# nwihardjo/SpaghettiSearch

Hardware: AMD Instinct MI355X
Metric: pagerank_iters_per_sec (higher is better)
Workload: dtype f64

## Files before the change

### include/spaghetti_rank.h

```cpp
#ifndef SPAGHETTI_RANK_H
#define SPAGHETTI_RANK_H

#include <stdint.h>

#ifdef __cplusplus
extern "C" {
#endif

#define SS_ABI_VERSION 4

enum {
    SS_OK = 0,
    SS_ERR_INVALID = 1,
    SS_ERR_NO_DEVICE = 2,
    SS_ERR_HIP = 3,
    SS_ERR_OOM = 4,
    SS_ERR_UNSORTED = 5,
    SS_ERR_STATE = 6,
    SS_ERR_UNSUPPORTED = 7,
    SS_ERR_COMM = 8
};

#define SS_MAX_TOPK 1024
#define SS_MAX_TOPICS 64
// ... 96 lines not shown
                       float* w_out, double* mag_out, float* idf_out);
int32_t ss_index_set_doc_freq(ss_index* idx, const uint64_t* df );
int32_t ss_index_set_weighted(ss_index* idx, const double* mag );
int32_t ss_index_set_positions(ss_index* idx, const uint64_t* pos_ptr, const float* pos);

int32_t ss_index_apply_delta(ss_index* idx, uint64_t n_del_docs, const uint32_t* del_docs,
                             uint64_t n_del, const uint32_t* del_term, const uint32_t* del_doc,
                             uint64_t n_add, const uint32_t* add_term, const uint32_t* add_doc, const float* add_w);
int32_t ss_index_apply_delta_pos(ss_index* idx, uint64_t n_del_docs, const uint32_t* del_docs,
                                 uint64_t n_del, const uint32_t* del_term, const uint32_t* del_doc,
                                 uint64_t n_add, const uint32_t* add_term, const uint32_t* add_doc, const float* add_w,
                                 const uint64_t* add_pos_ptr , const float* add_pos);
int32_t ss_index_resize(ss_index* idx, uint64_t n_docs_new, uint64_t n_terms_new);
int32_t ss_index_read_magnitudes(ss_index* idx, uint64_t n, const uint32_t* docs, double* mag_out);
int32_t ss_index_refresh_magnitudes(ss_index* idx, double* mag_out);
int32_t ss_index_get_info(const ss_index* idx, uint64_t* n_docs, uint64_t* n_terms, uint64_t* n_post);
int32_t ss_index_read(ss_index* idx, uint64_t* term_ptr_out , uint32_t* post_doc_out, float* post_w_out);
int32_t ss_index_read_positions(ss_index* idx, uint64_t* pos_ptr_out, float* pos_out);

int32_t ss_index_build_doc_view(ss_index* idx);
int32_t ss_index_drop_doc_view(ss_index* idx);
int32_t ss_index_read_doc_view(ss_index* idx, uint64_t* doc_ptr_out, uint32_t* doc_term_out, float* doc_w_out);
int32_t ss_index_doc_top_terms(ss_index* idx, uint64_t n, const uint32_t* docs , int32_t m,
                               uint32_t* terms_out , float* w_out , int32_t* n_out );

int32_t ss_scorer_create(ss_ctx* ctx, ss_index* title, ss_index* body, ss_scorer** out);
int32_t ss_scorer_destroy(ss_scorer* s);
int32_t ss_scorer_set_prior(ss_scorer* s, int32_t k_topics, const double* rank);
int32_t ss_score_topk(ss_scorer* s, int32_t n_q, const uint32_t* q_ptr, const uint32_t* q_terms,
                      const int32_t* query_len, const double* topic_probs, int32_t k,
// ... 196 lines not shown
```

### spaghettisearch_amd/_lib.py

```python
from __future__ import annotations

import ctypes as C
import os

_HERE = os.path.dirname(os.path.abspath(__file__))
LIB_PATH = os.environ.get("SS_LIB_PATH") or os.path.join(_HERE, "libspaghetti_rank.so")

SS_OK = 0
SS_MAX_TOPK = 1024
SS_MAX_TOPICS = 64
SS_MAX_QUERY_TERMS = 64
SS_MAX_FEEDBACK_DOCS = 64
SS_UNKNOWN_TERM = 0xFFFFFFFF
SS_NO_GROUP = 0xFFFFFFFF
SS_MAX_WORD_BYTES = 64
SS_MAX_EDIT_DIST = 3
SS_MAX_SUGGEST = 64
SS_MAX_SIG_SLOTS = 32
SS_SIG_EMPTY = 0xFFFFFFFF
SS_MAX_LINKS = 64
SS_LINKS_PARENTS = 0
SS_LINKS_CHILDREN = 1
SS_MAX_DOC_FIELDS = 4
SS_MAX_RANGE_CLAUSES = 4
# ... 95 lines not shown
    "ss_pr_exchange": (_i32, [_vp, _i32]),
    "ss_pagerank_run_sharded": (_i32, [_vp, _f64, _f64, _i32, _i32, _vp, _i32, _vp, _vp, _vp]),
    "ss_pagerank_run_group": (_i32, [_vp, _i32, _f64, _f64, _i32, _i32, _vp, _vp, _vp]),
    "ss_pr_status": (_i32, [_vp, _vp, C.POINTER(_i32), C.POINTER(_i32), _vp, _vp]),
    "ss_pr_read_local": (_i32, [_vp, _vp, _vp]),
    "ss_pr_read": (_i32, [_vp, _vp]),
    "ss_pr_probe": (_i32, [_vp, _i32, _i32, C.POINTER(C.c_float)]),
    "ss_index_create": (_i32, [_vp, _u64, _u64, _vp, _vp, _vp, C.POINTER(_vp)]),
    "ss_index_destroy": (_i32, [_vp]),
    "ss_tfidf_build": (_i32, [_vp, _u64, _vp, _vp, _vp]),
    "ss_index_apply_delta": (_i32, [_vp, _u64, _vp, _u64, _vp, _vp, _u64, _vp, _vp, _vp]),
    "ss_index_apply_delta_pos": (_i32, [_vp, _u64, _vp, _u64, _vp, _vp, _u64, _vp, _vp, _vp, _vp, _vp]),
    "ss_index_resize": (_i32, [_vp, _u64, _u64]),
    "ss_index_read_magnitudes": (_i32, [_vp, _u64, _vp, _vp]),
    "ss_index_refresh_magnitudes": (_i32, [_vp, _vp]),
    "ss_index_get_info": (_i32, [_vp, C.POINTER(_u64), C.POINTER(_u64), C.POINTER(_u64)]),
    "ss_index_read": (_i32, [_vp, _vp, _vp, _vp]),
    "ss_index_read_positions": (_i32, [_vp, _vp, _vp]),
    "ss_index_set_doc_freq": (_i32, [_vp, _vp]),
    "ss_index_set_weighted": (_i32, [_vp, _vp]),
    "ss_index_set_positions": (_i32, [_vp, _vp, _vp]),
    "ss_index_build_doc_view": (_i32, [_vp]),
    "ss_index_drop_doc_view": (_i32, [_vp]),
    "ss_index_read_doc_view": (_i32, [_vp, _vp, _vp, _vp]),
    "ss_index_doc_top_terms": (_i32, [_vp, _u64, _vp, _i32, _vp, _vp, _vp]),
    "ss_scorer_create": (_i32, [_vp, _vp, _vp, C.POINTER(_vp)]),
    "ss_scorer_destroy": (_i32, [_vp]),
    "ss_scorer_set_prior": (_i32, [_vp, _i32, _vp]),
    "ss_score_topk": (_i32, [_vp, _i32, _vp, _vp, _vp, _vp, _i32, _vp, _vp]),
    "ss_score_topk_phrase": (_i32, [_vp, _i32, _vp, _vp, _vp, _vp, _vp, _vp, _i32, _vp, _vp]),
# ... 76 lines not shown
```

### spaghettisearch_amd/csrc/ctx.hip

```cpp
#include "common.hpp"
#include <chrono>

#include <unordered_map>

namespace ss {

namespace {
struct Pool {
    std::mutex mu;
    std::multimap<std::pair<int, size_t>, void*> free_blocks;
    std::unordered_map<void*, std::pair<int, size_t>> live;
    size_t held = 0, limit = (size_t)64 << 30;
    double miss_ms = 0.0;
    uint64_t misses = 0;
    int contexts = 0;
};
Pool& pool() { static Pool* p = new Pool(); return *p; }
size_t size_class(size_t b) {
    if (b <= 4096) return 4096;
    size_t p2 = 4096;
    while (p2 < b) p2 <<= 1;
    if (p2 <= ((size_t)1 << 20)) return p2;
    const size_t step = p2 >> 4;
    return (b + step - 1) / step * step;
// ... 257 lines not shown
    "pr.lean_sweeps",
    "pr.item_turns",
    "graph.late_free",
    "graph.readback_runs",
    "pr.trace",
    "score.collect_pinned",
    "score.pipeline_slices",
    "score.timing",
    "score.trace",
    "pr.probe_hot",
    "pr.topic_blocks",
    "tfidf.blocks",
    "tfidf.bucket_shift",
    "tfidf.head_min_run",
    "tfidf.bucket_min",
    "score.wave",
    "score.wave_max_terms",
    "score.wave_min_list",
    "score.wave_share_pct",
    "score.wave_slice_target",
    "score.wave_big_pct",
    "score.wave_big_x100",
    "score.small",
    "score.small_max_batch",
    "score.small_batch",
    "score.small_cap",
    "score.pipeline",
    "score.grade_slices",
    "score.wave_small_x100",
    "score.exact_all",
// ... 55 lines not shown
```

### spaghettisearch_amd/csrc/index.hip

```cpp
#include "index.hpp"
#include <algorithm>
#include <memory>
#include <new>

namespace {

constexpr int TPB = 256;

__global__ void k_check_ptr(const uint64_t* __restrict__ term_ptr, uint64_t n_terms, const uint32_t* __restrict__ post_doc,
                            unsigned long long* __restrict__ n_boundary_desc, uint32_t* __restrict__ err) {
    const uint64_t t = (uint64_t)blockIdx.x * blockDim.x + threadIdx.x;
    if (t >= n_terms) return;
    const uint64_t a = term_ptr[t], b = term_ptr[t + 1];
    if (b < a) { atomicOr(err, 1u); return; }
    if (b > a && a > 0 && post_doc[a] <= post_doc[a - 1]) atomicAdd(n_boundary_desc, 1ull);
}
__global__ void k_check_df(const uint64_t* __restrict__ term_ptr, const uint64_t* __restrict__ df, uint64_t n_terms,
                           uint32_t* __restrict__ err) {
    const uint64_t t = (uint64_t)blockIdx.x * blockDim.x + threadIdx.x;
    if (t >= n_terms) return;
    if (df[t] < term_ptr[t + 1] - term_ptr[t]) atomicOr(err, 1u);
}
__global__ void k_check_pos(const uint64_t* __restrict__ pos_ptr, uint64_t n_post, uint32_t* __restrict__ err) {
    uint64_t i = (uint64_t)blockIdx.x * blockDim.x + threadIdx.x;
// ... 54 lines not shown
    SS_HIP(ctx, idx->mag2.alloc(n_docs));
    if (P) {
        SS_HIP(ctx, hipMemcpyAsync(idx->post_doc.p, post_doc, P * sizeof(uint32_t), hipMemcpyDefault, st));
        SS_HIP(ctx, hipMemcpyAsync(idx->post_w.p, post_tf, P * sizeof(float), hipMemcpyDefault, st));
    }
    SS_HIP(ctx, hipMemsetAsync(idx->mag.p, 0, n_docs * sizeof(double), st));

    ss::DevBuf<unsigned long long> d_cnt;
    ss::DevBuf<uint32_t> d_err;
    SS_HIP(ctx, d_cnt.alloc(2));
    SS_HIP(ctx, d_err.alloc(1));
    SS_HIP(ctx, hipMemsetAsync(d_cnt.p, 0, 2 * sizeof(unsigned long long), st));
    SS_HIP(ctx, hipMemsetAsync(d_err.p, 0, sizeof(uint32_t), st));
    if (n_terms) hipLaunchKernelGGL(k_check_ptr, dim3(ss::div_up(n_terms, TPB)), dim3(TPB), 0, st, idx->term_ptr.p, n_terms,
                                    idx->post_doc.p, d_cnt.p, d_err.p);
    if (P) hipLaunchKernelGGL(k_check_docs, dim3(std::min<unsigned>(ss::div_up(P, TPB), 16384u)), dim3(TPB), 0, st,
                              idx->post_doc.p, P, n_docs, d_cnt.p + 1, d_err.p);
    unsigned long long h_cnt[2] = {0, 0};
    uint32_t h_err = 0;
    SS_HIP(ctx, ss::fetch(ctx, st, h_cnt, d_cnt.p, sizeof(h_cnt), &h_err, d_err.p, sizeof(h_err)));
    SS_HIP(ctx, hipGetLastError());
    if (h_err & 1) return ctx->fail(SS_ERR_INVALID, "ss_index_create: term_ptr is not non-decreasing");
    if (h_err & 2) return ctx->fail(SS_ERR_INVALID, "ss_index_create: posting holds a doc id >= n_docs");
    if (h_cnt[1] != h_cnt[0])
        return ctx->fail(SS_ERR_UNSORTED, "ss_index_create: %llu posting(s) not strictly ascending by doc id inside a term",
                         h_cnt[1] - h_cnt[0]);
    *out = idx.release();
    return SS_OK;
}

int32_t ss_index_destroy(ss_index* idx) {
    if (!idx) return SS_ERR_INVALID;
// ... 2 lines not shown
    if (idx->users > 0) return ctx->fail(SS_ERR_STATE, "ss_index_destroy: index still used by %d scorer(s)", idx->users);
    (void)hipSetDevice(ctx->device);
    (void)hipStreamSynchronize(ctx->stream);
    delete idx;
    return SS_OK;
}

int32_t ss_index_get_info(const ss_index* idx, uint64_t* n_docs, uint64_t* n_terms, uint64_t* n_post) {
    if (!idx) return SS_ERR_INVALID;
    if (n_docs) *n_docs = idx->n_docs;
    if (n_terms) *n_terms = idx->n_terms;
    if (n_post) *n_post = idx->n_post;
    return SS_OK;
}

int32_t ss_index_read(ss_index* idx, uint64_t* term_ptr_out, uint32_t* post_doc_out, float* post_w_out) {
    if (!idx) return SS_ERR_INVALID;
    ss_ctx* ctx = idx->ctx;
    std::lock_guard<std::recursive_mutex> lk(ctx->mu);
    SS_HIP(ctx, hipSetDevice(ctx->device));
    hipStream_t st = ctx->stream;
    if (term_ptr_out) SS_HIP(ctx, hipMemcpyAsync(term_ptr_out, idx->term_ptr.p, (idx->n_terms + 1) * sizeof(uint64_t), hipMemcpyDefault, st));
    if (post_doc_out && idx->n_post) SS_HIP(ctx, hipMemcpyAsync(post_doc_out, idx->post_doc.p, idx->n_post * sizeof(uint32_t), hipMemcpyDefault, st));
    if (post_w_out && idx->n_post) SS_HIP(ctx, hipMemcpyAsync(post_w_out, idx->post_w.p, idx->n_post * sizeof(float), hipMemcpyDefault, st));
    SS_HIP(ctx, hipStreamSynchronize(st));
    return SS_OK;
}

int32_t ss_index_read_positions(ss_index* idx, uint64_t* pos_ptr_out, float* pos_out) {
    if (!idx) return SS_ERR_INVALID;
// ... 1 lines not shown
    std::lock_guard<std::recursive_mutex> lk(ctx->mu);
    if (!idx->pos_ptr.p) return ctx->fail(SS_ERR_STATE, "ss_index_read_positions: the table holds no positional postings");
    SS_HIP(ctx, hipSetDevice(ctx->device));
    hipStream_t st = ctx->stream;
    if (pos_ptr_out) SS_HIP(ctx, hipMemcpyAsync(pos_ptr_out, idx->pos_ptr.p, (idx->n_post + 1) * sizeof(uint64_t), hipMemcpyDefault, st));
    if (pos_out && idx->pos.n) SS_HIP(ctx, hipMemcpyAsync(pos_out, idx->pos.p, idx->pos.n * sizeof(float), hipMemcpyDefault, st));
    SS_HIP(ctx, hipStreamSynchronize(st));
    return SS_OK;
}

int32_t ss_index_set_doc_freq(ss_index* idx, const uint64_t* df) {
    if (!idx) return SS_ERR_INVALID;
    ss_ctx* ctx = idx->ctx;
    std::lock_guard<std::recursive_mutex> lk(ctx->mu);
    if (idx->weighted) return ctx->fail(SS_ERR_STATE, "ss_index_set_doc_freq: table is already weighted");
    if (!df) { idx->has_df_global = false; idx->df_global.release(); return SS_OK; }
    SS_HIP(ctx, hipSetDevice(ctx->device));
    hipStream_t st = ctx->stream;
    const uint64_t T = idx->n_terms;
    SS_HIP(ctx, idx->df_global.alloc(T));
    ss::DevBuf<uint32_t> err;
    SS_HIP(ctx, err.alloc(1));
    SS_HIP(ctx, hipMemsetAsync(err.p, 0, sizeof(uint32_t), st));
    if (T) {
        SS_HIP(ctx, hipMemcpyAsync(idx->df_global.p, df, T * sizeof(uint64_t), hipMemcpyDefault, st));
        hipLaunchKernelGGL(k_check_df, dim3(ss::div_up(T, TPB)), dim3(TPB), 0, st, idx->term_ptr.p, idx->df_global.p, T, err.p);
    }
    uint32_t h_err = 0;
    SS_HIP(ctx, ss::fetch(ctx, st, &h_err, err.p, sizeof(uint32_t)));
    if (h_err) {
// ... 52 lines not shown
```

### spaghettisearch_amd/csrc/index.hpp

```cpp
#pragma once
#include "common.hpp"

struct ss_index {
    ss_ctx* ctx = nullptr;
    uint64_t n_docs = 0, n_terms = 0, n_post = 0;
    ss::DevBuf<uint64_t> term_ptr;
    ss::DevBuf<uint32_t> post_doc;
    ss::DevBuf<float> post_w;
    ss::DevBuf<double> mag;
    ss::DevBuf<double> mag2;
    bool mag2_valid = false;
    ss::DevBuf<uint64_t> pos_ptr;
    ss::DevBuf<float> pos;
    ss::DevBuf<uint64_t> df_global;
    bool has_df_global = false;
    std::vector<uint64_t> h_term_ptr;
    bool weighted = false;
    int users = 0;
    ss::DevBuf<uint64_t> dv_ptr;
    ss::DevBuf<uint32_t> dv_term;
    ss::DevBuf<float> dv_w;
    bool has_doc_view = false;
    void drop_doc_view() {
        dv_ptr.release();
        dv_term.release();
        dv_w.release();
        has_doc_view = false;
    }
    ss::DevBuf<uint32_t> sig;
    int32_t sig_slots = 0;
    bool has_signatures = false;
    void drop_signatures() {
        sig.release();
        sig_slots = 0;
        has_signatures = false;
    }
};

namespace ss {
void launch_doc_top_terms(const ss_index* idx, const uint32_t* d_docs, uint64_t n, int32_t m, uint32_t* d_terms, float* d_w, int32_t* d_n, hipStream_t st);
}
```

### spaghettisearch_amd/csrc/index_update.hip

```cpp
#include "index.hpp"

#include <rocprim/rocprim.hpp>

#include <algorithm>
#include <memory>

namespace {

constexpr int TPB = 256;

inline unsigned grid_for(uint64_t n, unsigned cap = 1u << 16) { return (unsigned)std::min<uint64_t>(std::max<uint64_t>((n + TPB - 1) / TPB, 1), cap); }

__global__ void k_mark_docs(const uint32_t* __restrict__ del_docs, uint64_t n_del, uint64_t n_docs, uint32_t* __restrict__ bitmap, uint32_t* __restrict__ err) {
    for (uint64_t i = (uint64_t)blockIdx.x * blockDim.x + threadIdx.x; i < n_del; i += (uint64_t)gridDim.x * blockDim.x) {
        const uint32_t d = del_docs[i];
        if ((uint64_t)d >= n_docs) { atomicOr(err, 1u); continue; }
        atomicOr(&bitmap[d >> 5], 1u << (d & 31));
    }
}
__global__ void k_mark_touched(const uint32_t* __restrict__ docs, uint64_t n, uint64_t n_docs, uint32_t* __restrict__ touched) {
    for (uint64_t i = (uint64_t)blockIdx.x * blockDim.x + threadIdx.x; i < n; i += (uint64_t)gridDim.x * blockDim.x) {
        const uint32_t d = docs[i];
        if ((uint64_t)d < n_docs) atomicOr(&touched[d >> 5], 1u << (d & 31));
    }
// ... 424 lines not shown
            SS_HIP(ctx, rocprim::radix_sort_pairs(nullptr, tmp_bytes, t_keys_in.p, t_keys.p, t_sq_in.p, t_sq.p, (size_t)h_n, 0u, 64u, st));
            ss::DevBuf<char> tmp;
            SS_HIP(ctx, tmp.alloc(tmp_bytes));
            SS_HIP(ctx, rocprim::radix_sort_pairs(tmp.p, tmp_bytes, t_keys_in.p, t_keys.p, t_sq_in.p, t_sq.p, (size_t)h_n, 0u, 64u, st));
            SS_HIP(ctx, hipStreamSynchronize(st));
        }
        if (n_del_docs) hipLaunchKernelGGL(k_mag_zero_docs, dim3(grid_for(n_del_docs)), dim3(TPB), 0, st, (const uint32_t*)d_del_docs.p, n_del_docs, idx->mag2.p, idx->mag.p);
        if (n_del) hipLaunchKernelGGL(k_mag_zero_docs, dim3(grid_for(n_del)), dim3(TPB), 0, st, (const uint32_t*)d_del_doc.p, n_del, idx->mag2.p, idx->mag.p);
        if (n_add) hipLaunchKernelGGL(k_mag_zero_docs, dim3(grid_for(n_add)), dim3(TPB), 0, st, (const uint32_t*)d_add_doc.p, n_add, idx->mag2.p, idx->mag.p);
        if (h_n) hipLaunchKernelGGL(k_mag_segments, dim3(grid_for(h_n)), dim3(TPB), 0, st, (const uint64_t*)t_keys.p, (const float*)t_sq.p, (uint64_t)h_n, idx->mag2.p, idx->mag.p);
        SS_HIP(ctx, hipGetLastError());
    }
    SS_HIP(ctx, hipStreamSynchronize(st));
    idx->drop_doc_view();
    idx->drop_signatures();
    idx->post_doc = std::move(out_doc);
    idx->post_w = std::move(out_w);
    idx->term_ptr = std::move(new_ptr);
    idx->h_term_ptr = std::move(h_new_ptr);
    idx->n_post = P2;
    if (has_pos) {
        idx->pos_ptr = std::move(new_pos_ptr);
        idx->pos = std::move(new_pos);
    }
    return SS_OK;
}

int32_t ss_index_resize(ss_index* idx, uint64_t n_docs_new, uint64_t n_terms_new) {
    if (!idx) return SS_ERR_INVALID;
    ss_ctx* ctx = idx->ctx;
    std::lock_guard<std::recursive_mutex> lk(ctx->mu);
    if (idx->users > 0) return ctx->fail(SS_ERR_STATE, "ss_index_resize: %d scorer(s) still hold this table", idx->users);
    if (n_docs_new < idx->n_docs || n_terms_new < idx->n_terms) return ctx->fail(SS_ERR_INVALID, "ss_index_resize: a table only grows");
    if (n_docs_new >= 0xFFFFFFF0ull || n_terms_new >= 0xFFFFFFF0ull) return ctx->fail(SS_ERR_INVALID, "ss_index_resize: n_docs/n_terms out of range");
    if (idx->has_df_global && n_terms_new != idx->n_terms) return ctx->fail(SS_ERR_UNSUPPORTED, "ss_index_resize: a doc-range shard with whole-corpus document frequencies cannot grow its term space");
    SS_HIP(ctx, hipSetDevice(ctx->device));
    hipStream_t st = ctx->stream;
    const uint64_t T = idx->n_terms, N = idx->n_docs, P = idx->n_post;
    idx->drop_doc_view();
    idx->drop_signatures();
    if (n_terms_new > T) {
        ss::DevBuf<uint64_t> tp;
        SS_HIP(ctx, tp.alloc(n_terms_new + 1));
        SS_HIP(ctx, hipMemcpyAsync(tp.p, idx->term_ptr.p, (T + 1) * sizeof(uint64_t), hipMemcpyDeviceToDevice, st));
        hipLaunchKernelGGL(k_fill_u64, dim3(grid_for(n_terms_new - T)), dim3(TPB), 0, st, tp.p, T + 1, n_terms_new + 1, P);
        SS_HIP(ctx, hipStreamSynchronize(st));
        idx->term_ptr = std::move(tp);
        idx->h_term_ptr.resize(n_terms_new + 1, P);
        idx->n_terms = n_terms_new;
    }
    if (n_docs_new > N) {
        ss::DevBuf<double> m, m2;
        SS_HIP(ctx, m.alloc(n_docs_new));
        SS_HIP(ctx, m2.alloc(n_docs_new));
        SS_HIP(ctx, hipMemsetAsync(m.p, 0, n_docs_new * sizeof(double), st));
// ... 32 lines not shown
```

### spaghettisearch_amd/csrc/tfidf.hip

```cpp
#include "index.hpp"
#include "tfidf_plan.hpp"
#include <cstdlib>
#include <algorithm>

namespace {

using namespace ss::tfidf;

constexpr int TPB = 256;
static_assert(CH == TPB * 16, "k_weight and k_weight_count: 16 postings per thread");

__device__ __forceinline__ double go_log(double x) {
    const double Ln2Hi = 6.93147180369123816490e-01, Ln2Lo = 1.90821492927058770002e-10;
    const double L1 = 6.666666666666735130e-01, L2 = 3.999999999940941908e-01, L3 = 2.857142874366239149e-01,
                 L4 = 2.222219843214978396e-01, L5 = 1.818357216161805012e-01, L6 = 1.531383769920937332e-01,
                 L7 = 1.479819860511658591e-01;
    const double Sqrt2Half = 0.70710678118654752440084436210484903928483593768847;
    if (x != x || (isinf(x) && x > 0)) return x;
    if (x < 0) return __builtin_nan("");
    if (x == 0) return -__builtin_inf();
    int ki;
    double f1 = frexp(x, &ki);
    if (f1 < Sqrt2Half) { f1 *= 2; ki--; }
    const double f = f1 - 1;
// ... 184 lines not shown
#pragma unroll
                for (int j = 0; j < PER_THREAD; j++) {
                    const bool ok = x0 + j < n_here;
                    doc[j] = ok ? post_doc[i0 + j] : 0u;
                }
            }
#pragma unroll
            for (int j = 0; j < PER_THREAD; j++)
                if (x0 + j < n_here && !(nh && hk.hit(i0 + j))) atomicAdd(&s_hist[doc[j] >> shift], 1u);
        }
    }
    __syncthreads();
    for (uint32_t b = threadIdx.x; b < nb; b += TPB) mat[(size_t)b * nblk + blockIdx.x] = s_hist[b];
}

__global__ __launch_bounds__(64) void k_bucket_rowscan(uint32_t* __restrict__ mat, uint32_t nblk, uint32_t* __restrict__ cnt) {
    uint32_t* row = mat + (size_t)blockIdx.x * nblk;
    const uint32_t per = (nblk + 63) / 64, lane = threadIdx.x;
    uint32_t sum = 0;
    for (uint32_t j = 0; j < per; j++) {
        const uint32_t i = lane * per + j;
        if (i < nblk) sum += row[i];
    }
    uint32_t incl = sum;
#pragma unroll
    for (int off = 1; off < 64; off <<= 1) {
        const uint32_t v = __shfl_up(incl, off, 64);
        if ((int)lane >= off) incl += v;
    }
    uint32_t run = incl - sum;
    for (uint32_t j = 0; j < per; j++) {
        const uint32_t i = lane * per + j;
        if (i < nblk) { const uint32_t c = row[i]; row[i] = run; run += c; }
    }
    if (lane == 63) cnt[blockIdx.x] = incl;
}

__global__ __launch_bounds__(1024) void k_bucket_offsets(const uint32_t* __restrict__ cnt, uint32_t nb, uint32_t* __restrict__ off,
                                                         uint32_t* __restrict__ cursor) {
    __shared__ uint32_t s[NB_MAX];
    __shared__ uint32_t part[1024];
    const uint32_t per = (nb + 1023) / 1024;
    uint32_t sum = 0;
    for (uint32_t j = 0; j < per; j++) {
        const uint32_t b = threadIdx.x * per + j;
        const uint32_t c = b < nb ? cnt[b] : 0;
        if (b < nb) s[b] = sum;
        sum += c;
// ... 491 lines not shown
        SS_HIP(ctx, hipFuncSetAttribute(reinterpret_cast<const void*>(k_scatter<false, 2>), hipFuncAttributeMaxDynamicSharedMemorySize, lds));
        SS_HIP(ctx, hipFuncSetAttribute(reinterpret_cast<const void*>(k_scatter<true, 4>), hipFuncAttributeMaxDynamicSharedMemorySize, lds));
        SS_HIP(ctx, hipFuncSetAttribute(reinterpret_cast<const void*>(k_scatter<false, 4>), hipFuncAttributeMaxDynamicSharedMemorySize, lds));
        SS_HIP(ctx, hipFuncSetAttribute(reinterpret_cast<const void*>(k_scatter<true, SC_BPT_MAX>), hipFuncAttributeMaxDynamicSharedMemorySize, lds));
        SS_HIP(ctx, hipFuncSetAttribute(reinterpret_cast<const void*>(k_scatter<false, SC_BPT_MAX>), hipFuncAttributeMaxDynamicSharedMemorySize, lds));
        ctx->tfidf_scatter_lds = lds;
    }
    if (ctx->tfidf_bucket_lds < (int)plan.bucket_lds_bytes) {
        const int lds = (int)plan.bucket_lds_bytes;
        SS_HIP(ctx, hipFuncSetAttribute(reinterpret_cast<const void*>(k_bucket_sum<true>), hipFuncAttributeMaxDynamicSharedMemorySize, lds));
        SS_HIP(ctx, hipFuncSetAttribute(reinterpret_cast<const void*>(k_bucket_sum<false>), hipFuncAttributeMaxDynamicSharedMemorySize, lds));
        ctx->tfidf_bucket_lds = lds;
    }
    return SS_OK;
}
void bucket_pass_launch(ss_index* idx, hipStream_t st, BucketPass& bp, bool weight, const float* idf) {
    const uint64_t P = idx->n_post, N = idx->n_docs, T = idx->n_terms;
    const Plan& pl = bp.plan;
    HeadArgs head{nullptr, nullptr, nullptr, nullptr, nullptr};
    if (pl.head_thr && T) {
        (void)hipMemsetAsync(bp.h_n.p, 0, sizeof(uint32_t), st);
        (void)hipMemsetAsync(bp.h_hist.p, 0, HEAD_LEVELS * sizeof(uint32_t), st);
        hipLaunchKernelGGL(k_head_hist, dim3(ss::div_up(T, TPB)), dim3(TPB), 0, st, idx->term_ptr.p, T, pl.head_thr, bp.h_hist.p);
        hipLaunchKernelGGL(k_head_select, dim3(ss::div_up(T, TPB)), dim3(TPB), 0, st, idx->term_ptr.p, T, pl.head_thr, (const uint32_t*)bp.h_hist.p,
                           bp.h_n.p, bp.h_term.p);
        hipLaunchKernelGGL(k_head_sort, dim3(1), dim3(1024), 0, st, idx->term_ptr.p, bp.h_n.p, bp.h_term.p, bp.h_hs.p, bp.h_he.p);
        hipLaunchKernelGGL(k_head_bounds, dim3((pl.nb + 1) * (HEAD_CAP / 256)), dim3(256), 0, st, (const uint32_t*)idx->post_doc.p, (const uint32_t*)bp.h_n.p,
                           (const uint64_t*)bp.h_hs.p, (const uint64_t*)bp.h_he.p, pl.shift, pl.nb, bp.h_bounds.p);
        head = HeadArgs{bp.h_n.p, bp.h_term.p, bp.h_hs.p, bp.h_he.p, bp.h_bounds.p};
    }
    hipLaunchKernelGGL(k_weight_count, dim3(pl.nblk), dim3(TPB), 0, st, (const uint32_t*)idx->post_doc.p, P, pl.per, pl.shift, pl.nb, pl.nblk,
                       bp.mat.p, head);
    hipLaunchKernelGGL(k_bucket_rowscan, dim3(pl.nb), dim3(64), 0, st, bp.mat.p, pl.nblk, bp.cnt.p);
    hipLaunchKernelGGL(k_bucket_offsets, dim3(1), dim3(1024), 0, st, bp.cnt.p, pl.nb, bp.off.p, bp.cur.p);
#define SS_SCATTER_LAUNCH(W, B)                                                                                                                     \
    hipLaunchKernelGGL((k_scatter<W, B>), dim3(pl.nblk), dim3(SC_TPB), pl.scatter_lds_bytes, st, (const uint32_t*)idx->post_doc.p, idx->post_w.p, P, \
                       pl.per, pl.shift, pl.nb, pl.nblk, pl.bpt, pl.nbt, (const uint32_t*)bp.mat.p, (const uint32_t*)bp.off.p, bp.packed.p, head,   \
                       (const uint64_t*)idx->term_ptr.p, T, idf)
    if (weight) {
        if (pl.bpt_inst == 2) SS_SCATTER_LAUNCH(true, 2); else if (pl.bpt_inst == 4) SS_SCATTER_LAUNCH(true, 4); else SS_SCATTER_LAUNCH(true, SC_BPT_MAX);
    } else {
        if (pl.bpt_inst == 2) SS_SCATTER_LAUNCH(false, 2); else if (pl.bpt_inst == 4) SS_SCATTER_LAUNCH(false, 4); else SS_SCATTER_LAUNCH(false, SC_BPT_MAX);
    }
#undef SS_SCATTER_LAUNCH
#ifdef SS_SC_PHASES
    {
        unsigned long long h[8];
        (void)hipStreamSynchronize(st);
// ... 2 lines not shown
        for (int i = 0; i < 8; i++) tot += h[i];
        fprintf(stderr, "[k_scatter phases, %u blocks, cycles of wave 0 summed] wait-for-previous-write-out+barrier %.1f%%  window staged %.1f%%  weights %.1f%%  count %.1f%%  scan %.1f%%  "
                        "stage+next loads issued %.1f%%  write-out %.1f%%  loop top %.1f%%  (total %.3g cycles = %.1f k per block)\n", pl.nblk,
                100.0 * h[0] / tot, 100.0 * h[1] / tot, 100.0 * h[2] / tot, 100.0 * h[3] / tot, 100.0 * h[4] / tot, 100.0 * h[5] / tot, 100.0 * h[6] / tot, 100.0 * h[7] / tot,
                (double)tot, (double)tot / pl.nblk / 1e3);
        unsigned long long z[8] = {};
        (void)hipMemcpyToSymbol(HIP_SYMBOL(g_sc_ph), z, sizeof(z));
    }
#endif
    if (weight) hipLaunchKernelGGL(k_bucket_sum<true>, dim3(pl.nb), dim3(TPB_B), pl.bucket_lds_bytes, st, bp.packed.p, bp.off.p, N, pl.shift,
                                   idx->mag.p, idx->mag2.p, (const uint32_t*)idx->post_doc.p, idx->post_w.p, idf, head);
    else hipLaunchKernelGGL(k_bucket_sum<false>, dim3(pl.nb), dim3(TPB_B), pl.bucket_lds_bytes, st, bp.packed.p, bp.off.p, N, pl.shift,
                            idx->mag.p, idx->mag2.p, (const uint32_t*)idx->post_doc.p, idx->post_w.p, idf, head);
}

template <class Begin>
int32_t magnitude_pass(ss_index* idx, hipStream_t st, BucketPass& bp, bool weight, const float* idf, Begin begin) {
    ss_ctx* ctx = idx->ctx;
    const uint64_t P = idx->n_post, T = idx->n_terms, N = idx->n_docs;
    Options o;
    o.blocks = ctx->opt("tfidf.blocks", o.blocks);
    o.bucket_shift = ctx->opt("tfidf.bucket_shift", o.bucket_shift);
    o.head_min_run = ctx->opt("tfidf.head_min_run", o.head_min_run);
    o.bucket_min = ctx->opt("tfidf.bucket_min", o.bucket_min);
    const Plan plan = make_plan(N, P, o);
    if (plan.bucketed) SS_TRY(bucket_pass_prepare(ctx, P, plan, bp));
    SS_TRY(begin());
    if (plan.bucketed) {
        bucket_pass_launch(idx, st, bp, weight, idf);
        return SS_OK;
    }
    if (P && weight) hipLaunchKernelGGL(k_weight, dim3(ss::div_up(P, CH)), dim3(TPB), 0, st, idx->term_ptr.p, T, idx->post_doc.p,
                                        idx->post_w.p, idf, P, idx->mag.p);
    else if (P) hipLaunchKernelGGL(k_sumsq_atomic, dim3(std::min<unsigned>(ss::div_up(P, TPB), 16384u)), dim3(TPB), 0, st, (const uint32_t*)idx->post_doc.p,
                                   (const float*)idx->post_w.p, P, idx->mag.p);
    SS_HIP(ctx, hipMemcpyAsync(idx->mag2.p, idx->mag.p, N * sizeof(double), hipMemcpyDeviceToDevice, st));
    hipLaunchKernelGGL(k_sqrt, dim3(ss::div_up(N, TPB)), dim3(TPB), 0, st, idx->mag.p, N);
    return SS_OK;
}

}

extern "C" {

int32_t ss_tfidf_build(ss_index* idx, uint64_t total_docs, float* w_out, double* mag_out, float* idf_out) {
    if (!idx) return SS_ERR_INVALID;
    ss_ctx* ctx = idx->ctx;
    std::lock_guard<std::recursive_mutex> lk(ctx->mu);
    SS_HIP(ctx, hipSetDevice(ctx->device));
    hipStream_t st = ctx->stream;
    const uint64_t P = idx->n_post, T = idx->n_terms, N = idx->n_docs;
    idx->drop_doc_view();
    idx->drop_signatures();
    ss::DevBuf<float> idf;
    SS_HIP(ctx, idf.alloc(T));
// ... 40 lines not shown
```

### spaghettisearch_amd/csrc/tfidf_plan.hpp

```cpp
#pragma once

#include <algorithm>
#include <cstddef>
#include <cstdint>

namespace ss {
namespace tfidf {

constexpr int CH = 4096;
constexpr int NB_MAX = 4096;
#ifndef SS_SC_TPB
#define SS_SC_TPB 1024
#endif
constexpr int SC_TPB = SS_SC_TPB;
#ifndef SS_SC_PT
#define SS_SC_PT (8192 / SS_SC_TPB)
#endif
constexpr int SC_PT = SS_SC_PT;
constexpr int SC_CH = SC_TPB * SC_PT;
constexpr int SC_WIN = SC_CH;
constexpr int SC_PF = (1024 + SC_TPB - 1) / SC_TPB;
constexpr int SC_BPT_MAX = NB_MAX / SC_TPB;
#ifndef SS_HEAD_CAP
#define SS_HEAD_CAP 1024
// ... 45 lines not shown
    if (!p.bucketed) return p;
    const uint64_t unit = std::max<uint64_t>(SC_CH, CH);
    const uint64_t target_blocks = (uint64_t)std::max<int64_t>(1, o.blocks);
    p.per = std::max<uint64_t>(unit, div_up(div_up(n_post, target_blocks), unit) * unit);
    p.nblk = (uint32_t)div_up(n_post, p.per);
    p.head_thr = o.head_min_run > 0 ? std::max<uint64_t>((uint64_t)o.head_min_run * p.nb, 2 * unit + 1) : 0;
    p.bpt = ((uint32_t)div_up(p.nb, (uint32_t)SC_TPB) + 1u) & ~1u;
    p.nbt = (p.nb + 1u) & ~1u;
    p.too_many_buckets = p.bpt > (uint32_t)SC_BPT_MAX;
    p.bpt_inst = p.bpt <= 2 ? 2 : p.bpt <= 4 ? 4 : SC_BPT_MAX;
    p.scatter_lds_bytes = scatter_lds_bytes(p.nbt);
    p.bucket_lds_bytes = bucket_lds_bytes(p.shift);
    return p;
}

}
}
```

### spaghettisearch_amd/engine.py

```python
from __future__ import annotations

import ctypes as C
from typing import Optional, Sequence

import numpy as np

from . import _lib
from ._lib import SsGraphInfo, SsHit, SsPassage, SsTermMatch, check

HIT_DTYPE = np.dtype([("doc", "<u4"), ("_pad", "<u4"), ("title", "<f8"), ("body", "<f8"),
                      ("pagerank", "<f8"), ("final", "<f8")])

TERM_MATCH_DTYPE = np.dtype([("title_w", "<f4"), ("body_w", "<f4"), ("flags", "<u4"), ("body_pos", "<f4")])

PASSAGE_DTYPE = np.dtype([("start", "<f4"), ("last", "<f4"), ("n_distinct", "<u4"), ("n_occ", "<u4"), ("token_mask", "<u8")])

DOC_RANGE_DTYPE = np.dtype([("field", "<i4"), ("_pad", "<i4"), ("lo", "<i8"), ("hi", "<i8")])

VEC_HIT_DTYPE = np.dtype([("doc", "<u4"), ("score", "<i4")])

DIV_INFO_DTYPE = np.dtype([("rel", "<i4"), ("sim", "<i4")])

FUSED_DTYPE = np.dtype([("score", "<f8"), ("vec_score", "<i4"), ("lex_rank", "<u2"), ("vec_rank", "<u2")])
FUSE_RRF, FUSE_WEIGHTED = 0, 1
# ... 397 lines not shown
        out = np.zeros(int(docs.shape[0]), dtype=np.float64)
        check(self.ctx.lib.ss_index_read_magnitudes(self.h, int(docs.shape[0]), _ptr(docs), _ptr(out)), self.ctx.h)
        return out

    def read_positions(self):
        pp = np.zeros(self.n_post + 1, dtype=np.uint64)
        check(self.ctx.lib.ss_index_read_positions(self.h, _ptr(pp), None), self.ctx.h)
        pv = np.zeros(int(pp[-1]), dtype=np.float32)
        check(self.ctx.lib.ss_index_read_positions(self.h, None, _ptr(pv)), self.ctx.h)
        return pp, pv

    def refresh_magnitudes(self) -> np.ndarray:
        mag = np.zeros(self.n_docs, dtype=np.float64)
        check(self.ctx.lib.ss_index_refresh_magnitudes(self.h, _ptr(mag)), self.ctx.h)
        return mag

    def read(self):
        tp = np.zeros(self.n_terms + 1, dtype=np.uint64)
        pd = np.zeros(self.n_post, dtype=np.uint32)
        pw = np.zeros(self.n_post, dtype=np.float32)
        check(self.ctx.lib.ss_index_read(self.h, _ptr(tp), _ptr(pd), _ptr(pw)), self.ctx.h)
        return tp, pd, pw

    def build_doc_view(self) -> None:
        check(self.ctx.lib.ss_index_build_doc_view(self.h), self.ctx.h)

    def drop_doc_view(self) -> None:
        check(self.ctx.lib.ss_index_drop_doc_view(self.h), self.ctx.h)

    def read_doc_view(self):
# ... 874 lines not shown
```

Baseline: 21160.

## Fuse bucket histogram into index-create doc check and reuse it in tfidf pass

At index creation the doc-validation kernel is replaced by one that also builds the per-block bucket histogram, which is cached on the index with a plan signature. The tfidf magnitude pass then skips its counting kernel when the signature matches, feeding the stored histogram into the row scan. This targets tfidf build cost, not the pagerank loop, so the pagerank metric should be essentially unaffected. It adds a cached buffer, invalidation hooks on postings rewrites, and host-side head-set hashing.

```diff
diff --git a/include/spaghetti_rank.h b/include/spaghetti_rank.h
--- a/include/spaghetti_rank.h
+++ b/include/spaghetti_rank.h
@@ -134,6 +134,7 @@
 int32_t ss_index_resize(ss_index* idx, uint64_t n_docs_new, uint64_t n_terms_new);
 int32_t ss_index_read_magnitudes(ss_index* idx, uint64_t n, const uint32_t* docs, double* mag_out);
 int32_t ss_index_refresh_magnitudes(ss_index* idx, double* mag_out);
+int32_t ss_index_count_passes(ss_index* idx, int64_t* n_out);
 int32_t ss_index_get_info(const ss_index* idx, uint64_t* n_docs, uint64_t* n_terms, uint64_t* n_post);
 int32_t ss_index_read(ss_index* idx, uint64_t* term_ptr_out , uint32_t* post_doc_out, float* post_w_out);
 int32_t ss_index_read_positions(ss_index* idx, uint64_t* pos_ptr_out, float* pos_out);
diff --git a/spaghettisearch_amd/_lib.py b/spaghettisearch_amd/_lib.py
--- a/spaghettisearch_amd/_lib.py
+++ b/spaghettisearch_amd/_lib.py
@@ -133,6 +133,7 @@
     "ss_index_resize": (_i32, [_vp, _u64, _u64]),
     "ss_index_read_magnitudes": (_i32, [_vp, _u64, _vp, _vp]),
     "ss_index_refresh_magnitudes": (_i32, [_vp, _vp]),
+    "ss_index_count_passes": (_i32, [_vp, C.POINTER(C.c_int64)]),
     "ss_index_get_info": (_i32, [_vp, C.POINTER(_u64), C.POINTER(_u64), C.POINTER(_u64)]),
     "ss_index_read": (_i32, [_vp, _vp, _vp, _vp]),
     "ss_index_read_positions": (_i32, [_vp, _vp, _vp]),
diff --git a/spaghettisearch_amd/csrc/ctx.hip b/spaghettisearch_amd/csrc/ctx.hip
--- a/spaghettisearch_amd/csrc/ctx.hip
+++ b/spaghettisearch_amd/csrc/ctx.hip
@@ -295,6 +295,7 @@
     "tfidf.bucket_shift",
     "tfidf.head_min_run",
     "tfidf.bucket_min",
+    "tfidf.create_hist",
     "score.wave",
     "score.wave_max_terms",
     "score.wave_min_list",
diff --git a/spaghettisearch_amd/csrc/index.hip b/spaghettisearch_amd/csrc/index.hip
--- a/spaghettisearch_amd/csrc/index.hip
+++ b/spaghettisearch_amd/csrc/index.hip
@@ -92,8 +92,11 @@
     SS_HIP(ctx, hipMemsetAsync(d_err.p, 0, sizeof(uint32_t), st));
     if (n_terms) hipLaunchKernelGGL(k_check_ptr, dim3(ss::div_up(n_terms, TPB)), dim3(TPB), 0, st, idx->term_ptr.p, n_terms,
                                     idx->post_doc.p, d_cnt.p, d_err.p);
-    if (P) hipLaunchKernelGGL(k_check_docs, dim3(std::min<unsigned>(ss::div_up(P, TPB), 16384u)), dim3(TPB), 0, st,
-                              idx->post_doc.p, P, n_docs, d_cnt.p + 1, d_err.p);
+    ss::CreateHistTmp hist_tmp;
+    bool took_hist = false;
+    SS_TRY(ss::tfidf_check_docs_hist(idx.get(), st, d_cnt.p + 1, d_err.p, hist_tmp, &took_hist));
+    if (P && !took_hist) hipLaunchKernelGGL(k_check_docs, dim3(std::min<unsigned>(ss::div_up(P, TPB), 16384u)), dim3(TPB), 0, st,
+                                            idx->post_doc.p, P, n_docs, d_cnt.p + 1, d_err.p);
     unsigned long long h_cnt[2] = {0, 0};
     uint32_t h_err = 0;
     SS_HIP(ctx, ss::fetch(ctx, st, h_cnt, d_cnt.p, sizeof(h_cnt), &h_err, d_err.p, sizeof(h_err)));
@@ -126,6 +129,15 @@
     return SS_OK;
 }
 
+int32_t ss_index_count_passes(ss_index* idx, int64_t* n_out) {
+    if (!idx) return SS_ERR_INVALID;
+    ss_ctx* ctx = idx->ctx;
+    std::lock_guard<std::recursive_mutex> lk(ctx->mu);
+    if (!n_out) return ctx->fail(SS_ERR_INVALID, "ss_index_count_passes: n_out is NULL");
+    *n_out = idx->n_count_pass;
+    return SS_OK;
+}
+
 int32_t ss_index_read(ss_index* idx, uint64_t* term_ptr_out, uint32_t* post_doc_out, float* post_w_out) {
     if (!idx) return SS_ERR_INVALID;
     ss_ctx* ctx = idx->ctx;
@@ -157,6 +169,7 @@
     ss_ctx* ctx = idx->ctx;
     std::lock_guard<std::recursive_mutex> lk(ctx->mu);
     if (idx->weighted) return ctx->fail(SS_ERR_STATE, "ss_index_set_doc_freq: table is already weighted");
+    idx->drop_create_hist();
     if (!df) { idx->has_df_global = false; idx->df_global.release(); return SS_OK; }
     SS_HIP(ctx, hipSetDevice(ctx->device));
     hipStream_t st = ctx->stream;
diff --git a/spaghettisearch_amd/csrc/index.hpp b/spaghettisearch_amd/csrc/index.hpp
--- a/spaghettisearch_amd/csrc/index.hpp
+++ b/spaghettisearch_amd/csrc/index.hpp
@@ -1,5 +1,6 @@
 #pragma once
 #include "common.hpp"
+#include "tfidf_plan.hpp"
 
 struct ss_index {
     ss_ctx* ctx = nullptr;
@@ -35,8 +36,35 @@
         sig_slots = 0;
         has_signatures = false;
     }
+    ss::DevBuf<uint32_t> hist_mat;
+    ss::tfidf::PlanSig hist_sig;
+    uint64_t post_gen = 0;
+    ss::tfidf::HeadSet head_set;
+    uint64_t head_set_thr = 0, head_set_gen = ~0ull;
+    int64_t n_count_pass = 0;
+    void drop_create_hist() {
+        hist_mat.release();
+        hist_sig = ss::tfidf::PlanSig();
+    }
+    void postings_rewritten() {
+        post_gen++;
+        drop_create_hist();
+    }
+    const ss::tfidf::HeadSet& heads_for(uint64_t head_thr) {
+        if (head_set_gen != post_gen || head_set_thr != head_thr) {
+            head_set = ss::tfidf::head_set(h_term_ptr.data(), n_terms, head_thr);
+            head_set_thr = head_thr;
+            head_set_gen = post_gen;
+        }
+        return head_set;
+    }
 };
 
 namespace ss {
+struct CreateHistTmp {
+    DevBuf<uint32_t> h_n, h_hist, h_term;
+    DevBuf<uint64_t> h_hs, h_he;
+};
+int32_t tfidf_check_docs_hist(ss_index* idx, hipStream_t st, unsigned long long* d_desc, uint32_t* d_err, CreateHistTmp& tmp, bool* took);
 void launch_doc_top_terms(const ss_index* idx, const uint32_t* d_docs, uint64_t n, int32_t m, uint32_t* d_terms, float* d_w, int32_t* d_n, hipStream_t st);
 }
diff --git a/spaghettisearch_amd/csrc/index_update.hip b/spaghettisearch_amd/csrc/index_update.hip
--- a/spaghettisearch_amd/csrc/index_update.hip
+++ b/spaghettisearch_amd/csrc/index_update.hip
@@ -462,6 +462,7 @@
     SS_HIP(ctx, hipStreamSynchronize(st));
     idx->drop_doc_view();
     idx->drop_signatures();
+    idx->postings_rewritten();
     idx->post_doc = std::move(out_doc);
     idx->post_w = std::move(out_w);
     idx->term_ptr = std::move(new_ptr);
@@ -487,6 +488,7 @@
     const uint64_t T = idx->n_terms, N = idx->n_docs, P = idx->n_post;
     idx->drop_doc_view();
     idx->drop_signatures();
+    idx->postings_rewritten();
     if (n_terms_new > T) {
         ss::DevBuf<uint64_t> tp;
         SS_HIP(ctx, tp.alloc(n_terms_new + 1));
diff --git a/spaghettisearch_amd/csrc/tfidf.hip b/spaghettisearch_amd/csrc/tfidf.hip
--- a/spaghettisearch_amd/csrc/tfidf.hip
+++ b/spaghettisearch_amd/csrc/tfidf.hip
@@ -222,13 +222,71 @@
     for (uint32_t b = threadIdx.x; b < nb; b += TPB) mat[(size_t)b * nblk + blockIdx.x] = s_hist[b];
 }
 
-__global__ __launch_bounds__(64) void k_bucket_rowscan(uint32_t* __restrict__ mat, uint32_t nblk, uint32_t* __restrict__ cnt) {
+__global__ __launch_bounds__(TPB) void k_check_docs_hist(const uint32_t* __restrict__ post_doc, uint64_t n_post, uint64_t n_docs, uint64_t per, int shift,
+                                                         uint32_t nb, uint32_t nblk, uint32_t* __restrict__ mat, HeadArgs head,
+                                                         unsigned long long* __restrict__ n_desc, uint32_t* __restrict__ err) {
+    __shared__ uint32_t s_hist[NB_MAX];
+    for (uint32_t b = threadIdx.x; b < nb; b += TPB) s_hist[b] = 0;
+    const uint64_t r0 = (uint64_t)blockIdx.x * per, r1 = min(n_post, r0 + per);
+    const uint32_t nh = head.n ? *head.n : 0u;
+    uint32_t hcur = nh ? head_first(head, nh, r0) : 0u;
+    __syncthreads();
+    HeadSkip hk = nh ? HeadSkip{0ull, 0ull, 0ull, 0ull} : HeadSkip{~0ull, ~0ull, ~0ull, ~0ull};
+    unsigned long long local = 0;
+    bool bad = false;
+    for (uint64_t base = r0; base < r1; base += CH) {
+        const uint32_t n_here = (uint32_t)min((uint64_t)CH, r1 - base);
+        bool head_only = false;
+        if (nh) {
+            head_skip(head, nh, hcur, base, hk);
+            head_only = hk.a_lo <= base && hk.a_hi >= base + n_here;
+        }
+        const uint32_t x0 = threadIdx.x * PER_THREAD;
+        if (x0 < n_here) {
+            uint32_t doc[PER_THREAD];
+            const uint64_t i0 = base + x0;
+            uint32_t prev = i0 > 0 ? post_doc[i0 - 1] : 0u;
+            const bool full = x0 + PER_THREAD <= n_here;
+            if (full) {
+#pragma unroll
+                for (int v4 = 0; v4 < PER_THREAD / 4; v4++) {
+                    const uint4 d = *reinterpret_cast<const uint4*>(&post_doc[i0 + v4 * 4]);
+                    doc[v4 * 4] = d.x; doc[v4 * 4 + 1] = d.y; doc[v4 * 4 + 2] = d.z; doc[v4 * 4 + 3] = d.w;
+                }
+            } else {
+#pragma unroll
+                for (int j = 0; j < PER_THREAD; j++) {
+                    const bool ok = x0 + j < n_here;
+                    doc[j] = ok ? post_doc[i0 + j] : 0u;
+                }
+            }
+#pragma unroll
+            for (int j = 0; j < PER_THREAD; j++) {
+                if (x0 + j < n_here) {
+                    const uint32_t d = doc[j];
+                    if ((uint64_t)d >= n_docs) bad = true;
+                    else if (!head_only && !(nh && hk.hit(i0 + j))) atomicAdd(&s_hist[d >> shift], 1u);
+                    if (i0 + j > 0 && d <= prev) local++;
+                    prev = d;
+                }
+            }
+        }
+    }
+    __syncthreads();
+    for (uint32_t b = threadIdx.x; b < nb; b += TPB) mat[(size_t)b * nblk + blockIdx.x] = s_hist[b];
+    if (bad) atomicOr(err, 2u);
+    for (int off = 32; off > 0; off >>= 1) local += __shfl_xor(local, off, 64);
+    if ((threadIdx.x & 63) == 0 && local) atomicAdd(n_desc, local);
+}
+
+__global__ __launch_bounds__(64) void k_bucket_rowscan(const uint32_t* src, uint32_t* mat, uint32_t nblk, uint32_t* __restrict__ cnt) {
     uint32_t* row = mat + (size_t)blockIdx.x * nblk;
+    const uint32_t* in = src + (size_t)blockIdx.x * nblk;
     const uint32_t per = (nblk + 63) / 64, lane = threadIdx.x;
     uint32_t sum = 0;
     for (uint32_t j = 0; j < per; j++) {
         const uint32_t i = lane * per + j;
-        if (i < nblk) sum += row[i];
+        if (i < nblk) sum += in[i];
     }
     uint32_t incl = sum;
 #pragma unroll
@@ -239,7 +297,7 @@
     uint32_t run = incl - sum;
     for (uint32_t j = 0; j < per; j++) {
         const uint32_t i = lane * per + j;
-        if (i < nblk) { const uint32_t c = row[i]; row[i] = run; run += c; }
+        if (i < nblk) { const uint32_t c = in[i]; row[i] = run; run += c; }
     }
     if (lane == 63) cnt[blockIdx.x] = incl;
 }
@@ -761,24 +819,30 @@
     }
     return SS_OK;
 }
-void bucket_pass_launch(ss_index* idx, hipStream_t st, BucketPass& bp, bool weight, const float* idf) {
+void head_select_launch(const ss_index* idx, hipStream_t st, uint64_t thr, uint32_t* h_n, uint32_t* h_hist, uint32_t* h_term, uint64_t* h_hs, uint64_t* h_he) {
+    const uint64_t T = idx->n_terms;
+    (void)hipMemsetAsync(h_n, 0, sizeof(uint32_t), st);
+    (void)hipMemsetAsync(h_hist, 0, HEAD_LEVELS * sizeof(uint32_t), st);
+    hipLaunchKernelGGL(k_head_hist, dim3(ss::div_up(T, TPB)), dim3(TPB), 0, st, idx->term_ptr.p, T, thr, h_hist);
+    hipLaunchKernelGGL(k_head_select, dim3(ss::div_up(T, TPB)), dim3(TPB), 0, st, idx->term_ptr.p, T, thr, (const uint32_t*)h_hist, h_n, h_term);
+    hipLaunchKernelGGL(k_head_sort, dim3(1), dim3(1024), 0, st, idx->term_ptr.p, h_n, h_term, h_hs, h_he);
+}
+void bucket_pass_launch(ss_index* idx, hipStream_t st, BucketPass& bp, bool weight, const float* idf, const uint32_t* stored) {
     const uint64_t P = idx->n_post, N = idx->n_docs, T = idx->n_terms;
     const Plan& pl = bp.plan;
     HeadArgs head{nullptr, nullptr, nullptr, nullptr, nullptr};
     if (pl.head_thr && T) {
-        (void)hipMemsetAsync(bp.h_n.p, 0, sizeof(uint32_t), st);
-        (void)hipMemsetAsync(bp.h_hist.p, 0, HEAD_LEVELS * sizeof(uint32_t), st);
-        hipLaunchKernelGGL(k_head_hist, dim3(ss::div_up(T, TPB)), dim3(TPB), 0, st, idx->term_ptr.p, T, pl.head_thr, bp.h_hist.p);
-        hipLaunchKernelGGL(k_head_select, dim3(ss::div_up(T, TPB)), dim3(TPB), 0, st, idx->term_ptr.p, T, pl.head_thr, (const uint32_t*)bp.h_hist.p,
-                           bp.h_n.p, bp.h_term.p);
-        hipLaunchKernelGGL(k_head_sort, dim3(1), dim3(1024), 0, st, idx->term_ptr.p, bp.h_n.p, bp.h_term.p, bp.h_hs.p, bp.h_he.p);
+        head_select_launch(idx, st, pl.head_thr, bp.h_n.p, bp.h_hist.p, bp.h_term.p, bp.h_hs.p, bp.h_he.p);
         hipLaunchKernelGGL(k_head_bounds, dim3((pl.nb + 1) * (HEAD_CAP / 256)), dim3(256), 0, st, (const uint32_t*)idx->post_doc.p, (const uint32_t*)bp.h_n.p,
                            (const uint64_t*)bp.h_hs.p, (const uint64_t*)bp.h_he.p, pl.shift, pl.nb, bp.h_bounds.p);
         head = HeadArgs{bp.h_n.p, bp.h_term.p, bp.h_hs.p, bp.h_he.p, bp.h_bounds.p};
     }
-    hipLaunchKernelGGL(k_weight_count, dim3(pl.nblk), dim3(TPB), 0, st, (const uint32_t*)idx->post_doc.p, P, pl.per, pl.shift, pl.nb, pl.nblk,
-                       bp.mat.p, head);
-    hipLaunchKernelGGL(k_bucket_rowscan, dim3(pl.nb), dim3(64), 0, st, bp.mat.p, pl.nblk, bp.cnt.p);
+    if (!stored) {
+        hipLaunchKernelGGL(k_weight_count, dim3(pl.nblk), dim3(TPB), 0, st, (const uint32_t*)idx->post_doc.p, P, pl.per, pl.shift, pl.nb, pl.nblk,
+                           bp.mat.p, head);
+        idx->n_count_pass++;
+    }
+    hipLaunchKernelGGL(k_bucket_rowscan, dim3(pl.nb), dim3(64), 0, st, stored ? stored : (const uint32_t*)bp.mat.p, bp.mat.p, pl.nblk, bp.cnt.p);
     hipLaunchKernelGGL(k_bucket_offsets, dim3(1), dim3(1024), 0, st, bp.cnt.p, pl.nb, bp.off.p, bp.cur.p);
 #define SS_SCATTER_LAUNCH(W, B)                                                                                                                     \
     hipLaunchKernelGGL((k_scatter<W, B>), dim3(pl.nblk), dim3(SC_TPB), pl.scatter_lds_bytes, st, (const uint32_t*)idx->post_doc.p, idx->post_w.p, P, \
@@ -811,20 +875,28 @@
                             idx->mag.p, idx->mag2.p, (const uint32_t*)idx->post_doc.p, idx->post_w.p, idf, head);
 }
 
-template <class Begin>
-int32_t magnitude_pass(ss_index* idx, hipStream_t st, BucketPass& bp, bool weight, const float* idf, Begin begin) {
-    ss_ctx* ctx = idx->ctx;
-    const uint64_t P = idx->n_post, T = idx->n_terms, N = idx->n_docs;
+Options plan_options(const ss_ctx* ctx) {
     Options o;
     o.blocks = ctx->opt("tfidf.blocks", o.blocks);
     o.bucket_shift = ctx->opt("tfidf.bucket_shift", o.bucket_shift);
     o.head_min_run = ctx->opt("tfidf.head_min_run", o.head_min_run);
     o.bucket_min = ctx->opt("tfidf.bucket_min", o.bucket_min);
-    const Plan plan = make_plan(N, P, o);
+    return o;
+}
+
+template <class Begin>
+int32_t magnitude_pass(ss_index* idx, hipStream_t st, BucketPass& bp, bool weight, const float* idf, Begin begin) {
+    ss_ctx* ctx = idx->ctx;
+    const uint64_t P = idx->n_post, T = idx->n_terms, N = idx->n_docs;
+    const Plan plan = make_plan(N, P, plan_options(ctx));
     if (plan.bucketed) SS_TRY(bucket_pass_prepare(ctx, P, plan, bp));
+    const uint32_t* stored = nullptr;
+    if (plan.bucketed && idx->hist_sig.valid && ctx->opt("tfidf.create_hist", 1) != 0 &&
+        make_sig(plan, N, idx->post_gen, idx->heads_for(plan.head_thr)) == idx->hist_sig)
+        stored = idx->hist_mat.p;
     SS_TRY(begin());
     if (plan.bucketed) {
-        bucket_pass_launch(idx, st, bp, weight, idf);
+        bucket_pass_launch(idx, st, bp, weight, idf, stored);
         return SS_OK;
     }
     if (P && weight) hipLaunchKernelGGL(k_weight, dim3(ss::div_up(P, CH)), dim3(TPB), 0, st, idx->term_ptr.p, T, idx->post_doc.p,
@@ -836,6 +908,31 @@
     return SS_OK;
 }
 
+}
+
+int32_t ss::tfidf_check_docs_hist(ss_index* idx, hipStream_t st, unsigned long long* d_desc, uint32_t* d_err, CreateHistTmp& tmp, bool* took) {
+    *took = false;
+    ss_ctx* ctx = idx->ctx;
+    const uint64_t P = idx->n_post, T = idx->n_terms, N = idx->n_docs;
+    if (!P || ctx->opt("tfidf.create_hist", 1) == 0) return SS_OK;
+    const Plan plan = make_plan(N, P, plan_options(ctx));
+    if (!plan.bucketed || plan.too_many_buckets) return SS_OK;
+    SS_HIP(ctx, idx->hist_mat.alloc((size_t)plan.nb * plan.nblk));
+    HeadArgs head{nullptr, nullptr, nullptr, nullptr, nullptr};
+    if (plan.head_thr && T) {
+        SS_HIP(ctx, tmp.h_n.alloc(1));
+        SS_HIP(ctx, tmp.h_hist.alloc(HEAD_LEVELS));
+        SS_HIP(ctx, tmp.h_term.alloc(HEAD_CAP));
+        SS_HIP(ctx, tmp.h_hs.alloc(HEAD_CAP));
+        SS_HIP(ctx, tmp.h_he.alloc(HEAD_CAP));
+        head_select_launch(idx, st, plan.head_thr, tmp.h_n.p, tmp.h_hist.p, tmp.h_term.p, tmp.h_hs.p, tmp.h_he.p);
+        head = HeadArgs{tmp.h_n.p, tmp.h_term.p, tmp.h_hs.p, tmp.h_he.p, nullptr};
+    }
+    hipLaunchKernelGGL(k_check_docs_hist, dim3(plan.nblk), dim3(TPB), 0, st, (const uint32_t*)idx->post_doc.p, P, N, plan.per, plan.shift, plan.nb,
+                       plan.nblk, idx->hist_mat.p, head, d_desc, d_err);
+    idx->hist_sig = make_sig(plan, N, idx->post_gen, idx->heads_for(plan.head_thr));
+    *took = true;
+    return SS_OK;
 }
 
 extern "C" {
diff --git a/spaghettisearch_amd/csrc/tfidf_plan.hpp b/spaghettisearch_amd/csrc/tfidf_plan.hpp
--- a/spaghettisearch_amd/csrc/tfidf_plan.hpp
+++ b/spaghettisearch_amd/csrc/tfidf_plan.hpp
@@ -83,5 +83,62 @@
     return p;
 }
 
+
+struct HeadSet {
+    uint64_t thr_eff = 0;
+    uint32_t n = 0;
+    uint64_t hash = 0;
+};
+inline bool operator==(const HeadSet& a, const HeadSet& b) { return a.thr_eff == b.thr_eff && a.n == b.n && a.hash == b.hash; }
+
+inline HeadSet head_set(const uint64_t* term_ptr, uint64_t n_terms, uint64_t head_thr) {
+    HeadSet h;
+    if (!head_thr || !n_terms) return h;
+    uint32_t hist[HEAD_LEVELS] = {};
+    for (uint64_t t = 0; t < n_terms; t++) {
+        const uint64_t len = term_ptr[t + 1] - term_ptr[t];
+        for (int j = 0; j < HEAD_LEVELS && len >= (head_thr << j); j++) hist[j]++;
+    }
+    int j = 0;
+    while (j + 1 < HEAD_LEVELS && hist[j] > (uint32_t)HEAD_CAP) j++;
+    h.thr_eff = head_thr << j;
+    h.hash = 0xcbf29ce484222325ull;
+    for (uint64_t t = 0; t < n_terms; t++)
+        if (term_ptr[t + 1] - term_ptr[t] >= h.thr_eff) {
+            h.n++;
+            for (int b = 0; b < 4; b++) h.hash = (h.hash ^ ((t >> (8 * b)) & 0xFFu)) * 0x100000001b3ull;
+        }
+    return h;
+}
+
+struct PlanSig {
+    bool valid = false;
+    int shift = 0;
+    uint32_t nb = 0, nblk = 0;
+    uint64_t per = 0;
+    uint64_t head_thr = 0;
+    HeadSet head;
+    uint64_t n_docs = 0;
+    uint64_t post_gen = 0;
+};
+inline bool operator==(const PlanSig& a, const PlanSig& b) {
+    return a.valid && b.valid && a.shift == b.shift && a.nb == b.nb && a.nblk == b.nblk && a.per == b.per && a.head_thr == b.head_thr &&
+           a.head == b.head && a.n_docs == b.n_docs && a.post_gen == b.post_gen;
+}
+inline PlanSig make_sig(const Plan& p, uint64_t n_docs, uint64_t post_gen, const HeadSet& head) {
+    PlanSig s;
+    if (!p.bucketed || p.too_many_buckets) return s;
+    s.valid = true;
+    s.shift = p.shift;
+    s.nb = p.nb;
+    s.nblk = p.nblk;
+    s.per = p.per;
+    s.head_thr = p.head_thr;
+    s.head = head;
+    s.n_docs = n_docs;
+    s.post_gen = post_gen;
+    return s;
+}
+
 }
 }
diff --git a/spaghettisearch_amd/engine.py b/spaghettisearch_amd/engine.py
--- a/spaghettisearch_amd/engine.py
+++ b/spaghettisearch_amd/engine.py
@@ -435,6 +435,11 @@
         mag = np.zeros(self.n_docs, dtype=np.float64)
         check(self.ctx.lib.ss_index_refresh_magnitudes(self.h, _ptr(mag)), self.ctx.h)
         return mag
+
+    def count_passes(self) -> int:
+        n = C.c_int64(0)
+        check(self.ctx.lib.ss_index_count_passes(self.h, C.byref(n)), self.ctx.h)
+        return int(n.value)
 
     def read(self):
         tp = np.zeros(self.n_terms + 1, dtype=np.uint64)
```

Result: no change. 21060 (-0.5%).
